# brech1/keaki

Hardware: AMD Instinct MI355X
Metric: BN254 G1 scalar-mults/sec on 2^24-point MSM (per GPU) (higher is better)
Workload: dtype u32 limbs, 256-bit Montgomery modular integer (9 x 29-bit lazy limbs in the bucket kernel, 8 x 32 elsewhere)

## Files before the change

### keaki_amd/csrc/msm.hip.h

```cpp
#pragma once
#include <type_traits>
#include "bn254_curve.hip.h"
#include "fq29.hip.h"
#include "xyzz29.hip.h"
#include "jac29.hip.h"
#include "xyzz29_g2.hip.h"

namespace bn254 {

typedef uint16_t u16;
typedef u32 v4u_t __attribute__((ext_vector_type(4)));
constexpr u32 DIGIT_NONE = 0xFFFFFFFFu;
#ifndef STAMP
#define STAMP(cond, i) do { } while (0)
#endif

struct MsmShape {
  u32 n;
  u32 c;
  u32 W;
  u32 k;
  u32 stride;
};
KDEV u32 msm_width(const MsmShape& s, u32 w) { return w < s.k ? s.c : s.c - 1; }
// ... 750 lines not shown
  for (u32 sid = blockIdx.x; sid < total; sid += gridDim.x) {
    const u32 slot = hv_owner[sid];
    const u32 t = hv_bucket[slot];
    const u32 cnt = counts[t];
    const u32 lo = (sid - hv_first[slot]) * HEAVY_SLICE, hi = min(cnt, lo + HEAVY_SLICE);
    const BinMeta bm = v.bins[part_bin(v.ps, t)];
    Xyzz<F> acc = xyzz_inf<F>();
    u32 vbase = 0;
    for (u32 cb = 0; cb < bm.nch && vbase < hi; cb += 256) {
      const u32 c = cb + threadIdx.x;
      u32 s = 0, e = 0;
      if (c < bm.nch) { const u32 se = seg_word(v, t, bm, c); s = se & 0xFFFFu; e = se >> 16; }
      const u32 len = e - s;
      u32 tot;
      const u32 v0 = vbase + block_exclusive_scan(len, &tot), v1 = v0 + len;
      if (threadIdx.x == 0) nlist = 0;
      __syncthreads();
      if (len && v1 > lo && v0 < hi) {
        const u32 a0 = v0 > lo ? v0 : lo, a1 = v1 < hi ? v1 : hi;
        const u32 k = atomicAdd(&nlist, 1u);
        seg_pos[k] = bm.img_base + c * C2_CAP + s + (a0 - v0);
        seg_n[k] = a1 - a0;
      }
      __syncthreads();
      const u32 nl = nlist;
      for (u32 j = 0; j < nl; j++) {
        const u32 p0 = seg_pos[j], nn = seg_n[j];
        for (u32 q = threadIdx.x; q < nn; q += 256) {
          u32 en = v.sorted[p0 + q];
          Aff<F> p = points[en & 0x7FFFFFFFu];
          acc = xyzz_add_mixed(acc, aff_cneg(p, (en >> 31) != 0));
        }
      }
      __syncthreads();
      vbase += tot;
    }
    sh[threadIdx.x] = acc;
    __syncthreads();
    for (u32 o2 = 128; o2 > 0; o2 >>= 1) {
      if (threadIdx.x < o2) sh[threadIdx.x] = xyzz_add(sh[threadIdx.x], sh[threadIdx.x + o2]);
      __syncthreads();
    }
    if (threadIdx.x == 0) slices[sid] = sh[0];
    __syncthreads();
  }
}
struct Acc29 {
  v4u_t q[9];
};
KDEV void acc29_store(Acc29* dst, const U29& X, const U29& Y, const U29& ZZ, const U29& ZZZ, bool empty) {
  u32 w[36];
#pragma unroll
  for (int i = 0; i < 9; i++) { w[i] = empty ? 0u : X.l[i]; w[9 + i] = empty ? 0u : Y.l[i]; w[18 + i] = empty ? 0u : ZZ.l[i]; w[27 + i] = empty ? 0u : ZZZ.l[i]; }
#pragma unroll
  for (int i = 0; i < 9; i++) dst->q[i] = v4u_t{w[4 * i], w[4 * i + 1], w[4 * i + 2], w[4 * i + 3]};
}
KDEV bool acc29_load(const Acc29* src, U29& X, U29& Y, U29& ZZ, U29& ZZZ) {
  u32 w[36];
#pragma unroll
  for (int i = 0; i < 9; i++) { const v4u_t v = src->q[i]; w[4 * i] = v[0]; w[4 * i + 1] = v[1]; w[4 * i + 2] = v[2]; w[4 * i + 3] = v[3]; }
  u32 any = 0;
#pragma unroll
  for (int i = 0; i < 9; i++) { X.l[i] = w[i]; Y.l[i] = w[9 + i]; ZZ.l[i] = w[18 + i]; ZZZ.l[i] = w[27 + i]; any |= w[18 + i]; }
  return any == 0;
}
enum { HV_SET = 0, HV_ADD = 1, HV_SET29 = 2, HV_ADD29 = 3 };
template <class F>
__global__ void __launch_bounds__(64) k_msm_heavy_combine(const u32* __restrict__ counts, const HeavyList* __restrict__ hv, u32 hv_cap, u32 hv_slice_cap,
                                                          const u32* __restrict__ hv_bucket, const u32* __restrict__ hv_first,
                                                          const Xyzz<F>* __restrict__ slices, Xyzz<F>* __restrict__ buckets, u32 mode,
                                                          Acc29* __restrict__ state29) {
  __shared__ Xyzz<F> sh[64];
  const u32 nh = min(hv->n, hv_cap);
  for (u32 slot = blockIdx.x; slot < nh; slot += gridDim.x) {
    const u32 t = hv_bucket[slot], first = hv_first[slot];
    const u32 nsl = (counts[t] + HEAVY_SLICE - 1) / HEAVY_SLICE;
    Xyzz<F> acc = xyzz_inf<F>();
    for (u32 k = threadIdx.x; k < nsl; k += 64)
      if (first + k < hv_slice_cap) acc = xyzz_add(acc, slices[first + k]);
    sh[threadIdx.x] = acc;
    __syncthreads();
    for (u32 o = 32; o > 0; o >>= 1) {
      if (threadIdx.x < o) sh[threadIdx.x] = xyzz_add(sh[threadIdx.x], sh[threadIdx.x + o]);
      __syncthreads();
    }
    if (threadIdx.x == 0) {
      Xyzz<F> r = sh[0];
      if (mode == HV_ADD) r = xyzz_add(buckets[t], r);
      if constexpr (std::is_same<F, Fq>::value) {
        if (mode == HV_ADD29) {
          U29 X, Y, ZZ, ZZZ;
          if (!acc29_load(state29 + t, X, Y, ZZ, ZZZ)) r = xyzz_add(Xyzz<Fq>{u29_to_fq(X), u29_to_fq(Y), u29_to_fq(ZZ), u29_to_fq(ZZZ)}, r);
        }
        if (mode == HV_SET29 || mode == HV_ADD29)
          acc29_store(state29 + t, u29_from_fq(r.x), u29_from_fq(r.y), u29_from_fq(r.zz), u29_from_fq(r.zzz), xyzz_is_inf(r));
        else
          buckets[t] = r;
      } else {
        buckets[t] = r;
      }
    }
    __syncthreads();
  }
}
KDEV bool msm_bucket_is_heavy(u32 cnt) { return cnt >= HEAVY_MIN; }

template <class F>
__global__ void __launch_bounds__(256) k_msm_accumulate(const Aff<F>* __restrict__ points, SortView v, const u32* __restrict__ counts,
                                                        const u32* __restrict__ perm, u32 nbuckets_total, Xyzz<F>* __restrict__ buckets, u32 cont) {
  u32 lane = blockIdx.x * blockDim.x + threadIdx.x;
  if (lane >= nbuckets_total) return;
  u32 t = perm[lane];
  u32 cnt = counts[t];
  if (msm_bucket_is_heavy(cnt)) return;
  if (cont && cnt == 0) return;
  SegWalker sw;
  seg_init(sw, v, t);
  Xyzz<F> acc = xyzz_inf<F>();
  if (cont) acc = buckets[t];
  for (u32 k = 0; k < cnt; k++) {
    u32 e = seg_next(sw, v);
    Aff<F> p = points[e & 0x7FFFFFFFu];
    acc = xyzz_add_mixed(acc, aff_cneg(p, (e >> 31) != 0));
  }
  buckets[t] = acc;
}

template <int NT>
KDEV Aff<Fq> msm_load_row(const Aff<Fq>* __restrict__ p) {
  if constexpr (NT == 0) {
    return *p;
  } else {
    const v4u_t* s = reinterpret_cast<const v4u_t*>(p);
    const v4u_t w0 = __builtin_nontemporal_load(s), w1 = __builtin_nontemporal_load(s + 1), w2 = __builtin_nontemporal_load(s + 2),
                w3 = __builtin_nontemporal_load(s + 3);
    Aff<Fq> q;
#pragma unroll
    for (int i = 0; i < 4; i++) { q.x.l[i] = w0[i]; q.x.l[4 + i] = w1[i]; q.y.l[i] = w2[i]; q.y.l[4 + i] = w3[i]; }
    return q;
  }
}
#ifdef KEAKI_DIAG
static __global__ void k_diag_mask_rows(u32* __restrict__ sorted, size_t words, u32 mask) {
  for (size_t i = (size_t)blockIdx.x * blockDim.x + threadIdx.x; i < words; i += (size_t)gridDim.x * blockDim.x) {
    const u32 e = sorted[i];
    sorted[i] = (e & 0x80000000u) | (e & mask);
  }
}
#endif
enum { ACC_WHOLE = 0, ACC_FIRST = 1, ACC_MIDDLE = 2, ACC_LAST = 3 };
template <int NT, int MODE, int PF = 2>
static __global__ void __launch_bounds__(256, 3) k_msm_accumulate_g1_u29(const Aff<Fq>* __restrict__ points, SortView v,
                                                                      const u32* __restrict__ counts, const u32* __restrict__ perm,
                                                                      u32 nbuckets_total, Xyzz<Fq>* __restrict__ buckets,
                                                                      Acc29* __restrict__ state29) {
  u32 lane = blockIdx.x * blockDim.x + threadIdx.x;
  if (lane >= nbuckets_total) return;
  u32 t = perm[lane];
  u32 cnt = counts[t];
  if constexpr (MODE == ACC_LAST) {
    if (msm_bucket_is_heavy(cnt)) cnt = 0;
  } else {
    if (msm_bucket_is_heavy(cnt)) return;
  }
  if constexpr (MODE == ACC_MIDDLE) {
    if (cnt == 0) return;
  }
  SegWalker sw;
  SegWalkerQ sq;
  if constexpr (PF != 2) seg_init(sw, v, t);
  U29 X1, Y1, ZZ, ZZZ;
  bool empty = true;
  if constexpr (MODE == ACC_MIDDLE || MODE == ACC_LAST) empty = acc29_load(state29 + t, X1, Y1, ZZ, ZZZ);
  u32 e1 = 0, e2 = 0;
  Aff<Fq> q1;
  __shared__ __attribute__((aligned(16))) u32 idx_slots[PF == 2 ? IDXQ_NQ * IDXQ_PLANE : 4];
  __shared__ __attribute__((aligned(16))) u32 idx_park[PF == 2 ? 256 * SEGQ_PARK : 4];
  const u32* my_slot = idx_slots + threadIdx.x * 4;
  u32* wave_slots = idx_slots + (threadIdx.x & ~63u) * 4;
  u32* park = idx_park + threadIdx.x * SEGQ_PARK;
  if constexpr (PF == 2) {
    segq_init(sq, v, t, park);
    if (cnt > 0) {
      segq_advance(sq, v, t, park);
      segq_fetch(sq, v, wave_slots);
      asm volatile("s_waitcnt vmcnt(0)" ::: "memory");
      e1 = segq_next(sq, v, t, my_slot, wave_slots, park);
      if (cnt > 1) {
        asm volatile("s_waitcnt vmcnt(0)" ::: "memory");
        e2 = segq_next(sq, v, t, my_slot, wave_slots, park);
      }
    }
    q1 = msm_load_row<NT>(points + (e1 & 0x7FFFFFFFu));
  } else if constexpr (PF != 0) {
    e1 = cnt > 0 ? seg_next(sw, v) : 0u; e2 = cnt > 1 ? seg_next(sw, v) : 0u;
    q1 = msm_load_row<NT>(points + (e1 & 0x7FFFFFFFu));
  }
  for (u32 k = 0; k < cnt; k++) {
    u32 e;
    Aff<Fq> q;
    if constexpr (PF == 2) {
      e = e1;
      asm volatile("s_waitcnt vmcnt(0)" ::: "memory");
      q = q1;
#pragma unroll
      for (int i = 0; i < 8; i++) { asm volatile("" : "+v"(q.x.l[i])); asm volatile("" : "+v"(q.y.l[i])); }
      u32 e3 = 0;
      if (k + 2 < cnt) e3 = segq_next(sq, v, t, my_slot, wave_slots, park);
      e1 = e2;
      if (k + 1 < cnt) q1 = msm_load_row<NT>(points + (e1 & 0x7FFFFFFFu));
      e2 = e3;
    } else if constexpr (PF != 0) {
      e = e1;
      q = q1;
      e1 = e2;
      if (k + 1 < cnt) q1 = msm_load_row<NT>(points + (e1 & 0x7FFFFFFFu));
      if (k + 2 < cnt) e2 = seg_next(sw, v);
    } else {
      e = seg_next(sw, v);
      q = msm_load_row<NT>(points + (e & 0x7FFFFFFFu));
    }
    if (aff_is_inf(q)) continue;
    q.y = f_cneg(q.y, (e >> 31) != 0);
    const U29 X2 = u29_from_sat_shift5(q.x.l), Y2 = u29_from_sat_shift5(q.y.l);
    if (empty) {
      X1 = u29_mul(X2, u29_one());
      Y1 = u29_mul(Y2, u29_one());
      ZZ = u29_one();
      ZZZ = u29_one();
      empty = false;
      continue;
    }
    const U29 U2 = u29_mul(X2, ZZ), S2 = u29_mul(Y2, ZZZ);
    const U29 P = u29_sub(U2, X1, Q29::K16), R = u29_sub(S2, Y1, Q29::K4);
    if (u29_maybe_zero(P)) {
      if (u29_is_zero(P)) {
        if (u29_is_zero(R)) {
          Xyzz<Fq> d = xyzz_dbl_aff(q);
          X1 = u29_from_fq(d.x); Y1 = u29_from_fq(d.y); ZZ = u29_from_fq(d.zz); ZZZ = u29_from_fq(d.zzz);
        } else {
          empty = true;
        }
        continue;
      }
    }
    const U29 PP = u29_sqr(P), PPP = u29_mul(P, PP), Q = u29_mul(X1, PP);
    const U29 X3 = u29_sub3(u29_sqr(R), PPP, Q);
    const U29 T = u29_sub(Q, X3, Q29::K16);
    U29 NY1;
#pragma unroll
    for (int i = 0; i < 9; i++) NY1.l[i] = Q29::K2[i] - Y1.l[i];
    Y1 = u29_mul2(R, T, NY1, PPP);
    X1 = X3;
    ZZ = u29_mul(ZZ, PP);
    ZZZ = u29_mul(ZZZ, PPP);
  }
  u32 ts = t;
  asm volatile("" : "+v"(ts));
  if constexpr (MODE == ACC_FIRST || MODE == ACC_MIDDLE) {
    acc29_store(state29 + ts, X1, Y1, ZZ, ZZZ, empty);
  } else {
    Xyzz<Fq> out = xyzz_inf<Fq>();
    if (!empty) {
      out.x = u29_to_fq(X1); out.y = u29_to_fq(Y1); out.zz = u29_to_fq(ZZ); out.zzz = u29_to_fq(ZZZ);
    }
    buckets[ts] = out;
  }
}

template <int CONT>
static __global__ void __launch_bounds__(256, 2) k_msm_accumulate_g2_u29(const Aff<Fq2>* __restrict__ points, SortView v,
                                                                      const u32* __restrict__ counts, const u32* __restrict__ perm,
                                                                      u32 nbuckets_total, Xyzz<Fq2>* __restrict__ buckets) {
  u32 lane = blockIdx.x * blockDim.x + threadIdx.x;
  if (lane >= nbuckets_total) return;
  u32 t = perm[lane];
  u32 cnt = counts[t];
  if (msm_bucket_is_heavy(cnt)) return;
  if (CONT && cnt == 0) return;
  __shared__ __attribute__((aligned(16))) u32 idx_slots[IDXQ_NQ * IDXQ_PLANE];
  __shared__ __attribute__((aligned(16))) u32 idx_park[256 * SEGQ_PARK];
  const u32* my_slot = idx_slots + threadIdx.x * 4;
  u32* wave_slots = idx_slots + (threadIdx.x & ~63u) * 4;
  u32* park = idx_park + threadIdx.x * SEGQ_PARK;
  SegWalkerQ sq;
  segq_init(sq, v, t, park);
  X29G2 acc = x29g2_inf();
  if constexpr (CONT != 0) acc = x29g2_load(buckets[t]);
  if (cnt > 0) {
    segq_advance(sq, v, t, park);
    segq_fetch(sq, v, wave_slots);
  }
  for (u32 k = 0; k < cnt; k++) {
    asm volatile("s_waitcnt vmcnt(0)" ::: "memory");
    const u32 e = segq_next(sq, v, t, my_slot, wave_slots, park);
    Aff<Fq2> q = points[e & 0x7FFFFFFFu];
    x29g2_add_mixed(acc, aff_cneg(q, (e >> 31) != 0));
  }
  u32 ts = t;
  asm volatile("" : "+v"(ts));
  buckets[ts] = x29g2_store(acc);
}

template <class F>
__global__ void __launch_bounds__(64) k_msm_reduce(const Xyzz<F>* __restrict__ buckets, MsmShape s, u32 L, u32 chunks_per_window,
                                                   Xyzz<F>* __restrict__ partials) {
  u32 g = blockIdx.x * blockDim.x + threadIdx.x;
  if (g >= s.W * chunks_per_window) return;
  u32 w = g / chunks_per_window, t = g % chunks_per_window;
  u32 lo = t * L;
  const u32 Bw = msm_nbuckets(s, w);
  const Xyzz<F>* bk = buckets + msm_bucket_base(s, w);
  typedef TailOps<F> O;
  typename O::P run = O::inf(), ws = O::inf();
  for (u32 j = L; j-- > 0;) {
    if (lo + j < Bw) {
      run = O::add(run, O::load(bk[lo + j]));
      ws = O::add(ws, run);
    }
  }
  if (lo != 0 && lo < Bw) {
    typename O::P m = O::inf();
    for (int b = 31 - __clz(lo); b >= 0; b--) {
      m = O::dbl(m);
      if ((lo >> b) & 1) m = O::add(m, run);
    }
    ws = O::add(ws, m);
  }
  partials[g] = O::store(ws);
}

template <class F>
__global__ void __launch_bounds__(64) k_msm_partial_groups(const Xyzz<F>* __restrict__ in, u32 chunks_in, u32 G, u32 chunks_out,
                                                           Xyzz<F>* __restrict__ out) {
  typedef TailOps<F> O;
  __shared__ typename O::P sh[64];
  u32 w = blockIdx.y, x = blockIdx.x, l = threadIdx.x;
  typename O::P acc = O::inf();
  for (u32 t = x * G + l; t < (x + 1) * G && t < chunks_in; t += 64) acc = O::add(acc, O::load(in[(size_t)w * chunks_in + t]));
  sh[l] = acc;
  __syncthreads();
  for (u32 o = 32; o > 0; o >>= 1) {
    if (l < o) sh[l] = O::add(sh[l], sh[l + o]);
    __syncthreads();
  }
  if (l == 0) out[(size_t)w * chunks_out + x] = O::store(sh[0]);
}

template <class F> KDEV void store_norm_jac(F* out, const Xyzz<F>& p);
template <class F>
__global__ void __launch_bounds__(64) k_msm_window_finish(const Xyzz<F>* __restrict__ partials, MsmShape s, u32 chunks_per_window,
                                                          Xyzz<F>* __restrict__ window_sums, F* __restrict__ out_jac) {
  typedef TailOps<F> O;
  __shared__ typename O::P sh[64];
  u32 w = blockIdx.x, l = threadIdx.x;
  typename O::P acc = O::inf();
  for (u32 t = l; t < chunks_per_window; t += 64) acc = O::add(acc, O::load(partials[(size_t)w * chunks_per_window + t]));
  sh[l] = acc;
  __syncthreads();
  for (u32 o = 32; o > 0; o >>= 1) {
    if (l < o) sh[l] = O::add(sh[l], sh[l + o]);
    __syncthreads();
  }
  if (l == 0) {
    typename O::P r = sh[0];
    for (u32 k = 0, nd = msm_bit_offset(s, w); k < nd; k++) r = O::dbl(r);
    if (out_jac) store_norm_jac(out_jac, O::store(r));
    else window_sums[w] = O::store(r);
  }
}

template <class F> KDEV Aff<F> xyzz_to_aff_tail(const Xyzz<F>& p) { return xyzz_to_aff(p); }
template <> KDEV Aff<Fq> xyzz_to_aff_tail<Fq>(const Xyzz<Fq>& p) {
  if (xyzz_is_inf(p)) return aff_inf<Fq>();
  Fq izzz = fq_inv(p.zzz);
  Fq izz = fq_sqr(izzz) * fq_sqr(p.zz);
  return {p.x * izz, p.y * izzz};
}
template <class F>
KDEV void store_norm_jac(F* out, const Xyzz<F>& p) {
  Aff<F> a = xyzz_to_aff_tail(p);
  if (xyzz_is_inf(p)) {
    out[0] = f_one<F>(); out[1] = f_one<F>(); out[2] = f_zero<F>();
  } else {
    out[0] = a.x; out[1] = a.y; out[2] = f_one<F>();
  }
}
template <class F>
__global__ void __launch_bounds__(64) k_msm_final(const Xyzz<F>* __restrict__ window_sums, u32 W, F* __restrict__ out_jac) {
  if (threadIdx.x != 0 || blockIdx.x != 0) return;
  Xyzz<F> acc = xyzz_inf<F>();
  for (u32 w = 0; w < W; w++) acc = xyzz_add(acc, window_sums[w]);
  store_norm_jac(out_jac, acc);
}


template <class F>
__global__ void __launch_bounds__(64) k_msm_build_tables(const Aff<F>* __restrict__ points, u32 N, MsmShape s, Aff<F>* __restrict__ table) {
  u32 i = blockIdx.x * blockDim.x + threadIdx.x;
  if (i >= N) return;
  Aff<F> p = points[i];
  table[i] = p;
#pragma unroll 1
  for (u32 w = 1; w < s.W; w++) {
    Jac<F> j = jac_from_aff(p);
    for (u32 d = msm_width(s, w - 1); d > 0; d--) j = jac_dbl(j);
    p = jac_to_aff(j);
    table[(size_t)w * N + i] = p;
  }
}

constexpr u32 TABLE_MAX_W = 16;
static __global__ void __launch_bounds__(64) k_msm_build_tables_g1(const Aff<Fq>* __restrict__ points, u32 N, MsmShape s, Aff<Fq>* __restrict__ table) {
  u32 i = blockIdx.x * blockDim.x + threadIdx.x;
  if (i >= N) return;
  const Aff<Fq> p = points[i];
  table[i] = p;
  if (aff_is_inf(p)) {
    for (u32 w = 1; w < s.W; w++) table[(size_t)w * N + i] = p;
    return;
  }
  J29 j;
  j.x = u29_from_fq(p.x); j.y = u29_from_fq(p.y); j.z = u29_one();
  U29 zs[TABLE_MAX_W];
  U29 prod = u29_one();
#pragma unroll 1
  for (u32 w = 1; w < s.W; w++) {
    for (u32 d = msm_width(s, w - 1); d > 0; d--) j = j29_dbl(j);
    Aff<Fq> tmp = {u29_to_fq(j.x), u29_to_fq(j.y)};
    table[(size_t)w * N + i] = tmp;
#pragma unroll
    for (u32 k = 1; k < TABLE_MAX_W; k++) if (k == w) zs[k] = j.z;
    prod = u29_mul(prod, j.z);
  }
  U29 tinv = u29_from_fq(fq_inv(u29_to_fq(prod)));
#pragma unroll 1
  for (u32 w = s.W - 1; w >= 1; w--) {
    U29 pre = u29_one(), zw = u29_one();
#pragma unroll
    for (u32 k = 1; k < TABLE_MAX_W; k++) {
      if (k < w) pre = u29_mul(pre, zs[k]);
      if (k == w) zw = zs[k];
    }
    const U29 zinv = u29_mul(tinv, pre);
    tinv = u29_mul(tinv, zw);
    const U29 zi2 = u29_sqr(zinv), zi3 = u29_mul(zi2, zinv);
    const Aff<Fq> jxy = table[(size_t)w * N + i];
    Aff<Fq> a = {u29_to_fq(u29_mul(u29_from_sat_shift5(jxy.x.l), zi2)), u29_to_fq(u29_mul(u29_from_sat_shift5(jxy.y.l), zi3))};
    table[(size_t)w * N + i] = a;
  }
}

template <class F>
__global__ void __launch_bounds__(64) k_sum_jac(const F* __restrict__ pts, u32 k, F* __restrict__ out_jac) {
  if (threadIdx.x != 0 || blockIdx.x != 0) return;
  Xyzz<F> acc = xyzz_inf<F>();
  for (u32 i = 0; i < k; i++) {
    Jac<F> p = {pts[3 * i], pts[3 * i + 1], pts[3 * i + 2]};
    if (jac_is_inf(p)) continue;
    Aff<F> a = f_eq(p.z, f_one<F>()) ? Aff<F>{p.x, p.y} : jac_to_aff(p);
    acc = xyzz_add_mixed(acc, a);
  }
  store_norm_jac(out_jac, acc);
}

}
```

### keaki_amd/csrc/msm_host.hip.h

```cpp
#pragma once
#include <algorithm>
#include <functional>
#include <type_traits>
#include <vector>
#include "internal.h"
#include "msm.hip.h"

namespace keaki_internal {
using namespace bn254;

inline int choose_window(size_t n, int forced = 0) {
  if (forced >= 3 && forced <= 24) return forced;
  if (n < 32) return 3;
  double best = 1e300;
  int bc = 3;
  for (int c = 3; c <= 22; c++) {
    MsmPlan p = msm_make_plan(n, c);
    if (p.nb > ((size_t)PART_MAX_BINS << PART_MAX_FINE_SHIFT)) continue;
    double cost = (double)n * p.s.W + 2.8 * (double)p.nb;
    if ((double)p.nb < 131072.0) cost *= 131072.0 / (double)p.nb;
    if (cost < best) { best = cost; bc = c; }
  }
  return bc;
}

template <class F>
keaki_status msm_dev(keaki_hip_ctx* ctx, const Aff<F>* d_points, size_t srs_len, const void* d_scalars, size_t n, void* d_out_jac,
                     const Aff<F>* d_table = nullptr, int c_table = 0, const MsmPipe* pipe = nullptr) {
  if (!d_out_jac || (n && (!d_points || !d_scalars))) return fail(ctx, KEAKI_ERR_BAD_ARG, "msm: null pointer");
  if (n > srs_len) return fail(ctx, KEAKI_ERR_TOO_LARGE, "msm: %zu scalars but the SRS holds %zu points", n, srs_len);
  if (n >= (1ull << 31)) return fail(ctx, KEAKI_ERR_BAD_ARG, "msm: n must be < 2^31 per device");
  const bool shared = d_table != nullptr && (n * 2 > srs_len || ctx->tune.msm_short_tables != 0);
  const MsmPlan plan = shared ? msm_make_plan(n, c_table) : msm_make_plan(n, choose_window(n, ctx->tune.msm_c));
  MsmShape s = plan.s;
  MsmShape rs = s;
  size_t nb = plan.nb;
  if (shared) {
    s.stride = (u32)srs_len;
    u32 cr = 0;
    while ((1u << cr) < plan.max_b) cr++;
    rs.n = s.n; rs.c = cr; rs.W = 1; rs.k = 1; rs.stride = 0;
    nb = plan.max_b;
    d_points = d_table;
    if ((double)srs_len * s.W >= 2147483647.0) return fail(ctx, KEAKI_ERR_BAD_ARG, "msm: precomputed table index overflows 31 bits");
  }
  ctx->last_c = (int)s.c;
  if ((double)n * s.W >= 4294967295.0) return fail(ctx, KEAKI_ERR_BAD_ARG, "msm: n * windows overflows 32-bit positions");
  u32 L = sizeof(F) > sizeof(Fq) ? (plan.max_b >= 64 ? 8 : plan.max_b)
                                 : plan.max_b >= (1u << 21) ? 32 : plan.max_b >= (1u << 20) ? 16 : (plan.max_b >= 64 ? 8 : plan.max_b);
  if (ctx->tune.reduce_l >= 1 && ctx->tune.reduce_l <= 4096 && (u32)ctx->tune.reduce_l <= plan.max_b) L = (u32)ctx->tune.reduce_l;
  const u32 chunks = cdiv(plan.max_b, L);
  ST_TRY(reserve(ctx, ctx->wsums, (size_t)rs.W * sizeof(Xyzz<F>)));
  Xyzz<F>* wsums = (Xyzz<F>*)ctx->wsums.p;
  F* out = (F*)d_out_jac;
  hipStream_t st = ctx->stream;
  if (ctx->timing) (void)hipEventRecord(ctx->ev[0], st);
  if (n == 0) {
    hipLaunchKernelGGL((k_msm_final<F>), dim3(1), dim3(64), 0, st, (const Xyzz<F>*)wsums, 0u, out);
    return launch_check(ctx, "msm_final");
  }
  const size_t K = pipe ? pipe->ranges.size() : 1;
  if (pipe && K < 1) return fail(ctx, KEAKI_ERR_BAD_ARG, "msm: bad chunk bounds");
  struct Pass {
    size_t lo, m, pairs, max_chunks, cm_bytes, bt_bytes, bm_bytes, sg_bytes, ts_bytes;
    PartShape ps;
  };
  std::vector<Pass> passes(K);
  size_t w_digits = 0, w_sorted = 0, w_offsets = 0, w_cursor = 0, w_pairs = 0, w_total = 0;
  for (size_t j = 0; j < K; j++) {
    Pass& q = passes[j];
    q.lo = pipe ? pipe->ranges[j].first : 0;
    q.m = pipe ? pipe->ranges[j].second : n;
    if (q.m == 0 || q.lo > n || q.m > n - q.lo) return fail(ctx, KEAKI_ERR_BAD_ARG, "msm: bad chunk bounds");
    w_total += q.m;
    if (!part_make_shape(q.m, s.W, nb, &q.ps, ctx->tune.part_shift))
      return fail(ctx, KEAKI_ERR_BAD_ARG, "msm: %zu buckets / %u windows exceed the bucket sort's LDS budget (window too large)", nb, s.W);
    q.pairs = q.m * (size_t)s.W;
    q.max_chunks = part_max_chunks(q.pairs, q.ps.nbins);
    q.cm_bytes = (size_t)q.ps.nbins * q.ps.ntiles * sizeof(uint2);
    q.bt_bytes = ((size_t)q.ps.nbins * 4 + 15) & ~(size_t)15;
    q.bm_bytes = (size_t)q.ps.nbins * sizeof(BinMeta);
    q.sg_bytes = nb * sizeof(v4u_t);
    q.ts_bytes = (size_t)q.ps.ntiles * (q.ps.nbins + 1) * 2;
    w_digits = std::max(w_digits, (size_t)q.ps.ntiles * q.ps.te * 4);
    w_sorted = std::max(w_sorted, q.pairs * 4 + 64);
    w_offsets = std::max(w_offsets, q.max_chunks * q.ps.nf * 4);
    w_cursor = std::max(w_cursor, q.cm_bytes + q.bt_bytes + q.bm_bytes + q.sg_bytes + q.ts_bytes);
    w_pairs = std::max(w_pairs, q.pairs);
  }
  if (w_total != n) return fail(ctx, KEAKI_ERR_BAD_ARG, "msm: the chunks cover %zu of %zu pairs", w_total, n);
  bool u29 = false;
  if constexpr (std::is_same<F, Fq>::value) u29 = ctx->tune.acc_u29;
  if constexpr (std::is_same<F, Fq2>::value) u29 = ctx->tune.acc_u29_g2;
  bool lazy_state = K > 1 && u29 && std::is_same<F, Fq>::value;
  ST_TRY(reserve(ctx, ctx->digits, w_digits));
  ST_TRY(reserve(ctx, ctx->sorted, w_sorted));
  ST_TRY(reserve(ctx, ctx->hist, nb * 4));
  ST_TRY(reserve(ctx, ctx->offsets, w_offsets));
  ST_TRY(reserve(ctx, ctx->cursor, w_cursor));
  ST_TRY(reserve(ctx, ctx->buckets, nb * sizeof(Xyzz<F>)));
  ST_TRY(reserve(ctx, ctx->partials, ((size_t)rs.W * chunks + (size_t)rs.W * 256) * sizeof(Xyzz<F>)));
  ST_TRY(reserve(ctx, ctx->perm, nb * 4 + 2 * CNT_BINS * 4 + sizeof(HeavyList)));
  const u32 hv_cap = (u32)(w_pairs / HEAVY_MIN + 1), hv_slice_cap = (u32)(hv_cap + w_pairs / HEAVY_SLICE + 1);
  const size_t hv_hdr = ((2 * (size_t)hv_cap + hv_slice_cap) * 4 + 255) & ~(size_t)255;
  ST_TRY(reserve(ctx, ctx->heavy, hv_hdr + (size_t)hv_slice_cap * sizeof(Xyzz<F>)));
  if (lazy_state) {
    const keaki_status st29 = reserve(ctx, ctx->acc29, nb * sizeof(Acc29));
    if (st29 == KEAKI_ERR_OOM) { lazy_state = false; u29 = false; ctx->err.clear(); }
    else if (st29 != KEAKI_OK) return st29;
  }
  u32 *tiles = (u32*)ctx->digits.p, *sorted = (u32*)ctx->sorted.p, *hist = (u32*)ctx->hist.p;
  u32* segoff = (u32*)ctx->offsets.p;
  Xyzz<F>* buckets = (Xyzz<F>*)ctx->buckets.p;
  Xyzz<F>* partials = (Xyzz<F>*)ctx->partials.p;
  Acc29* state29 = lazy_state ? (Acc29*)ctx->acc29.p : nullptr;
  u32* perm = (u32*)ctx->perm.p;
  u32 *gstart = perm + nb, *ghist = gstart + CNT_BINS;
  HeavyList* hv = (HeavyList*)(ghist + CNT_BINS);
  u32 *hv_bucket = (u32*)ctx->heavy.p, *hv_first = hv_bucket + hv_cap, *hv_owner = hv_first + hv_cap;
  Xyzz<F>* hv_slices = (Xyzz<F>*)((char*)ctx->heavy.p + hv_hdr);
  for (size_t j = 0; j < K; j++) {
    const Pass& q = passes[j];
    const PartShape& ps = q.ps;
    if (pipe && pipe->stage) ST_TRY(pipe->stage(j));
    MsmShape sj = s;
    sj.n = (u32)q.m;
    const Fr* scal = (const Fr*)d_scalars + q.lo;
    const Aff<F>* pts = d_points + q.lo;
    const bool first = j == 0, last = j + 1 == K;
    uint2* cellmeta = (uint2*)ctx->cursor.p;
    u32* bin_total = (u32*)((char*)ctx->cursor.p + q.cm_bytes);
    BinMeta* bins = (BinMeta*)((char*)bin_total + q.bt_bytes);
    v4u_t* segtab = (v4u_t*)((char*)bins + q.bm_bytes);
    u16* tstart = (u16*)((char*)segtab + q.sg_bytes);
    {
      const dim3 g1(ps.ntiles < ctx->n_cu ? ps.ntiles : ctx->n_cu), b1(T1_THREADS);
#define KEAKI_TILE_SORT(WS) hipLaunchKernelGGL(k_tile_sort<WS>, g1, b1, 0, st, scal, sj, ps, tiles, tstart)
      switch (s.W) {
        case 11: KEAKI_TILE_SORT(11); break;
        case 12: KEAKI_TILE_SORT(12); break;
        case 13: KEAKI_TILE_SORT(13); break;
        case 14: KEAKI_TILE_SORT(14); break;
        case 15: KEAKI_TILE_SORT(15); break;
        case 16: KEAKI_TILE_SORT(16); break;
        default: KEAKI_TILE_SORT(0); break;
      }
#undef KEAKI_TILE_SORT
    }
    ST_TRY(launch_check(ctx, "tile_sort"));
    hipLaunchKernelGGL(k_cell_prefix, dim3(ps.nbins), dim3(1024), 0, st, (const u16*)tstart, ps, cellmeta, bin_total);
    hipLaunchKernelGGL(k_bin_scan, dim3(1), dim3(1024), 0, st, (const u32*)bin_total, ps.nbins, bins);
    {
#define KEAKI_CHUNK_SORT1(L, R, Q, M)                                                                                                                  \
  hipLaunchKernelGGL((k_chunk_sort<L, R, Q, M>), dim3(ps.nbins), dim3(C2_THREADS), 0, st, (const u32*)tiles, (const uint2*)cellmeta, (const BinMeta*)bins, sj, \
                     ps, (u32)nb, sorted, segtab, segoff, hist)
#define KEAKI_CHUNK_SORT(L, R, Q) do { if (ctx->tune.cs_masked) KEAKI_CHUNK_SORT1(L, R, Q, true); else KEAKI_CHUNK_SORT1(L, R, Q, false); } while (0)
      switch (ps.geom) {
        case 0: KEAKI_CHUNK_SORT(8, 1, 16); break;
        case 1: KEAKI_CHUNK_SORT(16, 1, 16); break;
        case 2: KEAKI_CHUNK_SORT(16, 2, 8); break;
        default: KEAKI_CHUNK_SORT(16, 4, 4); break;
      }
#undef KEAKI_CHUNK_SORT1
#undef KEAKI_CHUNK_SORT
    }
    ST_TRY(launch_check(ctx, "chunk_sort"));
#ifdef KEAKI_DIAG
    if (ctx->tune.diag_row_mask) hipLaunchKernelGGL(k_diag_mask_rows, dim3(4096), dim3(256), 0, st, sorted, (size_t)q.pairs, (u32)ctx->tune.diag_row_mask);
#endif
    const SortView view = {sorted, bins, segtab, segoff, ps};
    HIP_TRY(ctx, hipMemsetAsync(ghist, 0, CNT_BINS * 4 + sizeof(HeavyList), st));
    hipLaunchKernelGGL(k_cnt_hist, dim3(cdiv(nb, 1024)), dim3(256), 0, st, (const u32*)hist, (u32)nb, ghist, hv, hv_cap, hv_slice_cap, hv_bucket, hv_first,
                       hv_owner);
    hipLaunchKernelGGL(k_cnt_offsets, dim3(1), dim3(CNT_BINS), 0, st, (const u32*)ghist, gstart);
    hipLaunchKernelGGL(k_cnt_scatter, dim3(cdiv(nb, 1024)), dim3(256), 0, st, (const u32*)hist, (u32)nb, gstart, perm);
    ST_TRY(launch_check(ctx, "cnt_sort"));
    if (ctx->timing && last) (void)hipEventRecord(ctx->ev[1], st);
    const dim3 ga(cdiv(nb, 256)), ba(256);
    bool done = false;
    if constexpr (std::is_same<F, Fq>::value) {
      if (u29) {
#define KEAKI_ACC(NT, MODE) hipLaunchKernelGGL((k_msm_accumulate_g1_u29<NT, MODE>), ga, ba, 0, st, pts, view, (const u32*)hist, (const u32*)perm, (u32)nb, buckets, state29)
        if (K == 1) {
          if (ctx->tune.acc_nt) KEAKI_ACC(1, ACC_WHOLE);
          else if (!ctx->tune.acc_prefetch)
            hipLaunchKernelGGL((k_msm_accumulate_g1_u29<0, ACC_WHOLE, 0>), ga, ba, 0, st, pts, view, (const u32*)hist, (const u32*)perm, (u32)nb, buckets, state29);
          else if (!ctx->tune.acc_idxq)
            hipLaunchKernelGGL((k_msm_accumulate_g1_u29<0, ACC_WHOLE, 1>), ga, ba, 0, st, pts, view, (const u32*)hist, (const u32*)perm, (u32)nb, buckets, state29);
          else KEAKI_ACC(0, ACC_WHOLE);
        }
        else if (first) KEAKI_ACC(0, ACC_FIRST);
        else if (!last) KEAKI_ACC(0, ACC_MIDDLE);
        else KEAKI_ACC(0, ACC_LAST);
#undef KEAKI_ACC
        done = true;
      }
    }
    if constexpr (std::is_same<F, Fq2>::value) {
      if (u29) {
        if (first) hipLaunchKernelGGL(k_msm_accumulate_g2_u29<0>, ga, ba, 0, st, pts, view, (const u32*)hist, (const u32*)perm, (u32)nb, buckets);
        else hipLaunchKernelGGL(k_msm_accumulate_g2_u29<1>, ga, ba, 0, st, pts, view, (const u32*)hist, (const u32*)perm, (u32)nb, buckets);
        done = true;
      }
    }
    if (!done)
      hipLaunchKernelGGL((k_msm_accumulate<F>), ga, ba, 0, st, pts, view, (const u32*)hist, (const u32*)perm, (u32)nb, buckets, first ? 0u : 1u);
    ST_TRY(launch_check(ctx, "msm_accumulate"));
    const u32 hv_mode = lazy_state && !last ? (first ? HV_SET29 : HV_ADD29) : (first ? HV_SET : HV_ADD);
    hipLaunchKernelGGL((k_msm_heavy<F>), dim3(HEAVY_GRID), dim3(256), 0, st, pts, view, (const u32*)hist,
                       (const HeavyList*)hv, hv_slice_cap, (const u32*)hv_bucket, (const u32*)hv_first, (const u32*)hv_owner, hv_slices);
    hipLaunchKernelGGL((k_msm_heavy_combine<F>), dim3(HEAVY_COMBINE_GRID), dim3(64), 0, st, (const u32*)hist, (const HeavyList*)hv, hv_cap, hv_slice_cap,
                       (const u32*)hv_bucket, (const u32*)hv_first, (const Xyzz<F>*)hv_slices, buckets, hv_mode, state29);
    ST_TRY(launch_check(ctx, "msm_heavy"));
  }
  if (ctx->timing) (void)hipEventRecord(ctx->ev[2], st);
  hipLaunchKernelGGL((k_msm_reduce<F>), dim3(cdiv((size_t)rs.W * chunks, 64)), dim3(64), 0, st, (const Xyzz<F>*)buckets, rs, L, chunks, partials);
  const Xyzz<F>* fin_in = partials;
  u32 fin_chunks = chunks;
  if (chunks > 256) {
    const u32 G = cdiv(chunks, 128);
    const u32 chunks2 = cdiv(chunks, G);
    Xyzz<F>* partials2 = partials + (size_t)rs.W * chunks;
    hipLaunchKernelGGL((k_msm_partial_groups<F>), dim3(chunks2, rs.W), dim3(64), 0, st, (const Xyzz<F>*)partials, chunks, G, chunks2, partials2);
    fin_in = partials2; fin_chunks = chunks2;
  }
  hipLaunchKernelGGL((k_msm_window_finish<F>), dim3(rs.W), dim3(64), 0, st, fin_in, rs, fin_chunks, wsums, rs.W == 1 ? out : (F*)nullptr);
  if (rs.W != 1) hipLaunchKernelGGL((k_msm_final<F>), dim3(1), dim3(64), 0, st, (const Xyzz<F>*)wsums, rs.W, out);
  ST_TRY(launch_check(ctx, "msm_reduce/final"));
  if (ctx->timing) {
    (void)hipEventRecord(ctx->ev[3], st);
    ctx->timing_pending = true;
  }
  return KEAKI_OK;
}

template <class F>
keaki_status msm_build_tables(keaki_hip_ctx* ctx, const Aff<F>* d_points, size_t N, int c_table, Aff<F>* d_table) {
  MsmPlan plan = msm_make_plan(N, c_table);
  bool done = false;
  if constexpr (std::is_same<F, Fq>::value) {
    if (plan.s.W <= TABLE_MAX_W) {
      hipLaunchKernelGGL(k_msm_build_tables_g1, dim3(cdiv(N, 64)), dim3(64), 0, ctx->stream, d_points, (u32)N, plan.s, d_table);
      done = true;
    }
  }
  if (!done)
  hipLaunchKernelGGL((k_msm_build_tables<F>), dim3(cdiv(N, 64)), dim3(64), 0, ctx->stream, d_points, (u32)N, plan.s, d_table);
  return launch_check(ctx, "msm_build_tables");
}
inline int choose_window_shared(size_t n, int forced = 0) {
  if (forced >= 3 && forced <= 24) return forced;
  double best = 1e300;
  int bc = 8;
  for (int c = 8; c <= 23; c++) {
    MsmPlan p = msm_make_plan(n, c);
    if (p.max_b > ((size_t)PART_MAX_BINS << PART_MAX_FINE_SHIFT)) continue;
    double cost = (double)n * p.s.W + 2.8 * (double)p.max_b;
    if ((double)p.max_b < 131072.0) cost *= 131072.0 / (double)p.max_b;
    if (cost < best) { best = cost; bc = c; }
  }
  return bc;
}
inline u32 msm_plan_windows(size_t n, int c) { return msm_make_plan(n, c).s.W; }

}
```

Before: 1.023 billion.

## Replace running-sum bucket reduction with bit-decomposed row/column line sums

Replaces the per-chunk running-sum bucket reduction with a bit-decomposition scheme. Bucket indices are laid out as a 2D grid, and partial row and column line sums are computed and then combined. For each bit of the index, the lines whose coordinate has that bit set are summed and doubled the matching number of times. This avoids the serial run/ws chains and the per-chunk double-and-add correction, and exposes more parallelism in the reduction tail. The cost is four kernel launches and a different partial buffer layout, with a new tunable T reusing the reduce_l knob.

```diff
diff --git a/keaki_amd/csrc/msm.hip.h b/keaki_amd/csrc/msm.hip.h
--- a/keaki_amd/csrc/msm.hip.h
+++ b/keaki_amd/csrc/msm.hip.h
@@ -1076,72 +1076,117 @@
   buckets[ts] = x29g2_store(acc);
 }
 
+struct TailGeom {
+  u32 lb, h;
+  u32 nr, nc;
+  u32 tr, tc;
+  u32 gc, gf;
+  u32 sc, sr;
+  u32 o_pr, o_c, o_r, o_u, per_w;
+};
+constexpr u32 TAIL_LINE_LANES = 16;
+inline TailGeom tail_geom(u32 max_b, u32 t) {
+  TailGeom g;
+  g.lb = 0;
+  while ((1u << g.lb) < max_b) g.lb++;
+  g.h = (g.lb + 1) / 2;
+  g.nr = 1u << (g.lb - g.h); g.nc = 1u << g.h;
+  g.tr = t < g.nr ? t : g.nr; g.tc = t < g.nc ? t : g.nc;
+  g.gc = (g.nr + g.tr - 1) / g.tr; g.gf = (g.nc + g.tc - 1) / g.tc;
+  g.sc = 1; while (g.sc * 2 <= g.gc && g.sc < TAIL_LINE_LANES) g.sc *= 2;
+  g.sr = 1; while (g.sr * 2 <= g.gf && g.sr < TAIL_LINE_LANES) g.sr *= 2;
+  g.o_pr = g.nc * g.gc; g.o_c = g.o_pr + g.nr * g.gf; g.o_r = g.o_c + g.nc; g.o_u = g.o_r + g.nr; g.per_w = g.o_u + g.lb + 1;
+  return g;
+}
+KDEV u32 tree_top(u32 m) { return m <= 1 ? 0u : 1u << (31 - __clz(m - 1)); }
+KDEV u32 umin(u32 a, u32 b) { return a < b ? a : b; }
+
 template <class F>
-__global__ void __launch_bounds__(64) k_msm_reduce(const Xyzz<F>* __restrict__ buckets, MsmShape s, u32 L, u32 chunks_per_window,
-                                                   Xyzz<F>* __restrict__ partials) {
-  u32 g = blockIdx.x * blockDim.x + threadIdx.x;
-  if (g >= s.W * chunks_per_window) return;
-  u32 w = g / chunks_per_window, t = g % chunks_per_window;
-  u32 lo = t * L;
+__global__ void __launch_bounds__(64) k_msm_tail_lines(const Xyzz<F>* __restrict__ buckets, MsmShape s, TailGeom g, Xyzz<F>* __restrict__ ws) {
+  typedef TailOps<F> O;
+  const u32 t = blockIdx.x * 64 + threadIdx.x, w = blockIdx.y;
+  if (t >= g.o_c) return;
+  u32 j0, step, len;
+  if (t < g.o_pr) {
+    const u32 b = t & (g.nc - 1), r0 = (t >> g.h) * g.tr;
+    j0 = (r0 << g.h) + b; step = g.nc; len = umin(g.tr, g.nr - r0);
+  } else {
+    const u32 u = t - g.o_pr, a = u & (g.nr - 1), c0 = (u >> (g.lb - g.h)) * g.tc;
+    j0 = (a << g.h) + c0; step = 1; len = umin(g.tc, g.nc - c0);
+  }
   const u32 Bw = msm_nbuckets(s, w);
-  const Xyzz<F>* bk = buckets + msm_bucket_base(s, w);
-  typedef TailOps<F> O;
-  typename O::P run = O::inf(), ws = O::inf();
-  for (u32 j = L; j-- > 0;) {
-    if (lo + j < Bw) {
-      run = O::add(run, O::load(bk[lo + j]));
-      ws = O::add(ws, run);
-    }
-  }
-  if (lo != 0 && lo < Bw) {
-    typename O::P m = O::inf();
-    for (int b = 31 - __clz(lo); b >= 0; b--) {
-      m = O::dbl(m);
-      if ((lo >> b) & 1) m = O::add(m, run);
-    }
-    ws = O::add(ws, m);
-  }
-  partials[g] = O::store(ws);
+  len = j0 >= Bw ? 0u : umin(len, (Bw - j0 + step - 1) / step);
+  const Xyzz<F>* bk = buckets + msm_bucket_base(s, w) + j0;
+  typename O::P acc = O::inf();
+  for (u32 i = 0; i < len; i++) acc = O::add(acc, O::load(bk[(size_t)i * step]));
+  ws[(size_t)w * g.per_w + t] = O::store(acc);
 }
 
 template <class F>
-__global__ void __launch_bounds__(64) k_msm_partial_groups(const Xyzz<F>* __restrict__ in, u32 chunks_in, u32 G, u32 chunks_out,
-                                                           Xyzz<F>* __restrict__ out) {
+__global__ void __launch_bounds__(64) k_msm_tail_line_sums(TailGeom g, Xyzz<F>* __restrict__ ws) {
   typedef TailOps<F> O;
   __shared__ typename O::P sh[64];
-  u32 w = blockIdx.y, x = blockIdx.x, l = threadIdx.x;
+  const u32 l = threadIdx.x, cb = (g.nc * g.sc + 63) / 64;
+  const bool col = blockIdx.x < cb;
+  const u32 span = col ? g.sc : g.sr, np = col ? g.gc : g.gf, nl = col ? g.nc : g.nr;
+  const u32 q = (col ? blockIdx.x : blockIdx.x - cb) * 64 + l, line = q / span, k = q % span;
+  Xyzz<F>* base = ws + (size_t)blockIdx.y * g.per_w;
+  const Xyzz<F>* in = base + (col ? 0u : g.o_pr);
   typename O::P acc = O::inf();
-  for (u32 t = x * G + l; t < (x + 1) * G && t < chunks_in; t += 64) acc = O::add(acc, O::load(in[(size_t)w * chunks_in + t]));
+  if (line < nl)
+    for (u32 i = k; i < np; i += span) acc = O::add(acc, O::load(in[(size_t)i * nl + line]));
   sh[l] = acc;
   __syncthreads();
-  for (u32 o = 32; o > 0; o >>= 1) {
+  for (u32 o = span >> 1; o > 0; o >>= 1) {
+    if (k < o) sh[l] = O::add(sh[l], sh[l + o]);
+    __syncthreads();
+  }
+  if (k == 0 && line < nl) base[(col ? g.o_c : g.o_r) + line] = O::store(sh[l]);
+}
+
+constexpr u32 TAIL_BITS_THREADS = 256;
+template <class F>
+__global__ void __launch_bounds__(TAIL_BITS_THREADS) k_msm_tail_bits(MsmShape s, TailGeom g, Xyzz<F>* __restrict__ ws) {
+  typedef TailOps<F> O;
+  __shared__ typename O::P sh[TAIL_BITS_THREADS];
+  const u32 e = blockIdx.x, w = blockIdx.y, l = threadIdx.x;
+  Xyzz<F>* base = ws + (size_t)w * g.per_w;
+  const bool colside = e < g.h, all = e == g.lb;
+  const Xyzz<F>* in = base + (colside ? g.o_c : g.o_r);
+  const u32 bit = colside ? e : e - g.h, cnt = all ? g.nr : (colside ? g.nc : g.nr) >> 1;
+  typename O::P acc = O::inf();
+  for (u32 i = l; i < cnt; i += TAIL_BITS_THREADS) {
+    const u32 x = all ? i : ((i >> bit) << (bit + 1)) | (1u << bit) | (i & ((1u << bit) - 1u));
+    acc = O::add(acc, O::load(in[x]));
+  }
+  sh[l] = acc;
+  __syncthreads();
+  for (u32 o = tree_top(umin(cnt, TAIL_BITS_THREADS)); o > 0; o >>= 1) {
     if (l < o) sh[l] = O::add(sh[l], sh[l + o]);
     __syncthreads();
   }
-  if (l == 0) out[(size_t)w * chunks_out + x] = O::store(sh[0]);
+  if (l == 0) {
+    typename O::P r = sh[0];
+    for (u32 d = (all ? 0u : e) + msm_bit_offset(s, w); d > 0; d--) r = O::dbl(r);
+    base[g.o_u + e] = O::store(r);
+  }
 }
 
 template <class F> KDEV void store_norm_jac(F* out, const Xyzz<F>& p);
 template <class F>
-__global__ void __launch_bounds__(64) k_msm_window_finish(const Xyzz<F>* __restrict__ partials, MsmShape s, u32 chunks_per_window,
-                                                          Xyzz<F>* __restrict__ window_sums, F* __restrict__ out_jac) {
+__global__ void __launch_bounds__(64) k_msm_tail_final(TailGeom g, u32 W, const Xyzz<F>* __restrict__ ws, F* __restrict__ out_jac) {
   typedef TailOps<F> O;
   __shared__ typename O::P sh[64];
-  u32 w = blockIdx.x, l = threadIdx.x;
+  const u32 l = threadIdx.x, per = g.lb + 1, cnt = W * per;
   typename O::P acc = O::inf();
-  for (u32 t = l; t < chunks_per_window; t += 64) acc = O::add(acc, O::load(partials[(size_t)w * chunks_per_window + t]));
+  for (u32 i = l; i < cnt; i += 64) acc = O::add(acc, O::load(ws[(size_t)(i / per) * g.per_w + g.o_u + i % per]));
   sh[l] = acc;
   __syncthreads();
-  for (u32 o = 32; o > 0; o >>= 1) {
+  for (u32 o = tree_top(umin(cnt, 64u)); o > 0; o >>= 1) {
     if (l < o) sh[l] = O::add(sh[l], sh[l + o]);
     __syncthreads();
   }
-  if (l == 0) {
-    typename O::P r = sh[0];
-    for (u32 k = 0, nd = msm_bit_offset(s, w); k < nd; k++) r = O::dbl(r);
-    if (out_jac) store_norm_jac(out_jac, O::store(r));
-    else window_sums[w] = O::store(r);
-  }
+  if (l == 0) store_norm_jac(out_jac, O::store(sh[0]));
 }
 
 template <class F> KDEV Aff<F> xyzz_to_aff_tail(const Xyzz<F>& p) { return xyzz_to_aff(p); }
@@ -1160,15 +1205,6 @@
     out[0] = a.x; out[1] = a.y; out[2] = f_one<F>();
   }
 }
-template <class F>
-__global__ void __launch_bounds__(64) k_msm_final(const Xyzz<F>* __restrict__ window_sums, u32 W, F* __restrict__ out_jac) {
-  if (threadIdx.x != 0 || blockIdx.x != 0) return;
-  Xyzz<F> acc = xyzz_inf<F>();
-  for (u32 w = 0; w < W; w++) acc = xyzz_add(acc, window_sums[w]);
-  store_norm_jac(out_jac, acc);
-}
-
-
 template <class F>
 __global__ void __launch_bounds__(64) k_msm_build_tables(const Aff<F>* __restrict__ points, u32 N, MsmShape s, Aff<F>* __restrict__ table) {
   u32 i = blockIdx.x * blockDim.x + threadIdx.x;
diff --git a/keaki_amd/csrc/msm_host.hip.h b/keaki_amd/csrc/msm_host.hip.h
--- a/keaki_amd/csrc/msm_host.hip.h
+++ b/keaki_amd/csrc/msm_host.hip.h
@@ -46,17 +46,14 @@
   }
   ctx->last_c = (int)s.c;
   if ((double)n * s.W >= 4294967295.0) return fail(ctx, KEAKI_ERR_BAD_ARG, "msm: n * windows overflows 32-bit positions");
-  u32 L = sizeof(F) > sizeof(Fq) ? (plan.max_b >= 64 ? 8 : plan.max_b)
-                                 : plan.max_b >= (1u << 21) ? 32 : plan.max_b >= (1u << 20) ? 16 : (plan.max_b >= 64 ? 8 : plan.max_b);
-  if (ctx->tune.reduce_l >= 1 && ctx->tune.reduce_l <= 4096 && (u32)ctx->tune.reduce_l <= plan.max_b) L = (u32)ctx->tune.reduce_l;
-  const u32 chunks = cdiv(plan.max_b, L);
-  ST_TRY(reserve(ctx, ctx->wsums, (size_t)rs.W * sizeof(Xyzz<F>)));
-  Xyzz<F>* wsums = (Xyzz<F>*)ctx->wsums.p;
+  u32 T = 22;
+  if (ctx->tune.reduce_l >= 1 && ctx->tune.reduce_l <= 4096) T = (u32)ctx->tune.reduce_l;
+  const TailGeom tg = tail_geom(plan.max_b, T);
   F* out = (F*)d_out_jac;
   hipStream_t st = ctx->stream;
   if (ctx->timing) (void)hipEventRecord(ctx->ev[0], st);
   if (n == 0) {
-    hipLaunchKernelGGL((k_msm_final<F>), dim3(1), dim3(64), 0, st, (const Xyzz<F>*)wsums, 0u, out);
+    hipLaunchKernelGGL((k_msm_tail_final<F>), dim3(1), dim3(64), 0, st, tg, 0u, (const Xyzz<F>*)nullptr, out);
     return launch_check(ctx, "msm_final");
   }
   const size_t K = pipe ? pipe->ranges.size() : 1;
@@ -99,7 +96,7 @@
   ST_TRY(reserve(ctx, ctx->offsets, w_offsets));
   ST_TRY(reserve(ctx, ctx->cursor, w_cursor));
   ST_TRY(reserve(ctx, ctx->buckets, nb * sizeof(Xyzz<F>)));
-  ST_TRY(reserve(ctx, ctx->partials, ((size_t)rs.W * chunks + (size_t)rs.W * 256) * sizeof(Xyzz<F>)));
+  ST_TRY(reserve(ctx, ctx->partials, (size_t)rs.W * tg.per_w * sizeof(Xyzz<F>)));
   ST_TRY(reserve(ctx, ctx->perm, nb * 4 + 2 * CNT_BINS * 4 + sizeof(HeavyList)));
   const u32 hv_cap = (u32)(w_pairs / HEAVY_MIN + 1), hv_slice_cap = (u32)(hv_cap + w_pairs / HEAVY_SLICE + 1);
   const size_t hv_hdr = ((2 * (size_t)hv_cap + hv_slice_cap) * 4 + 255) & ~(size_t)255;
@@ -112,7 +109,6 @@
   u32 *tiles = (u32*)ctx->digits.p, *sorted = (u32*)ctx->sorted.p, *hist = (u32*)ctx->hist.p;
   u32* segoff = (u32*)ctx->offsets.p;
   Xyzz<F>* buckets = (Xyzz<F>*)ctx->buckets.p;
-  Xyzz<F>* partials = (Xyzz<F>*)ctx->partials.p;
   Acc29* state29 = lazy_state ? (Acc29*)ctx->acc29.p : nullptr;
   u32* perm = (u32*)ctx->perm.p;
   u32 *gstart = perm + nb, *ghist = gstart + CNT_BINS;
@@ -214,19 +210,12 @@
     ST_TRY(launch_check(ctx, "msm_heavy"));
   }
   if (ctx->timing) (void)hipEventRecord(ctx->ev[2], st);
-  hipLaunchKernelGGL((k_msm_reduce<F>), dim3(cdiv((size_t)rs.W * chunks, 64)), dim3(64), 0, st, (const Xyzz<F>*)buckets, rs, L, chunks, partials);
-  const Xyzz<F>* fin_in = partials;
-  u32 fin_chunks = chunks;
-  if (chunks > 256) {
-    const u32 G = cdiv(chunks, 128);
-    const u32 chunks2 = cdiv(chunks, G);
-    Xyzz<F>* partials2 = partials + (size_t)rs.W * chunks;
-    hipLaunchKernelGGL((k_msm_partial_groups<F>), dim3(chunks2, rs.W), dim3(64), 0, st, (const Xyzz<F>*)partials, chunks, G, chunks2, partials2);
-    fin_in = partials2; fin_chunks = chunks2;
-  }
-  hipLaunchKernelGGL((k_msm_window_finish<F>), dim3(rs.W), dim3(64), 0, st, fin_in, rs, fin_chunks, wsums, rs.W == 1 ? out : (F*)nullptr);
-  if (rs.W != 1) hipLaunchKernelGGL((k_msm_final<F>), dim3(1), dim3(64), 0, st, (const Xyzz<F>*)wsums, rs.W, out);
-  ST_TRY(launch_check(ctx, "msm_reduce/final"));
+  Xyzz<F>* tws = (Xyzz<F>*)ctx->partials.p;
+  hipLaunchKernelGGL((k_msm_tail_lines<F>), dim3(cdiv(tg.o_c, 64), rs.W), dim3(64), 0, st, (const Xyzz<F>*)buckets, rs, tg, tws);
+  hipLaunchKernelGGL((k_msm_tail_line_sums<F>), dim3(cdiv((size_t)tg.nc * tg.sc, 64) + cdiv((size_t)tg.nr * tg.sr, 64), rs.W), dim3(64), 0, st, tg, tws);
+  hipLaunchKernelGGL((k_msm_tail_bits<F>), dim3(tg.lb + 1, rs.W), dim3(TAIL_BITS_THREADS), 0, st, rs, tg, tws);
+  hipLaunchKernelGGL((k_msm_tail_final<F>), dim3(1), dim3(64), 0, st, tg, rs.W, (const Xyzz<F>*)tws, out);
+  ST_TRY(launch_check(ctx, "msm_tail"));
   if (ctx->timing) {
     (void)hipEventRecord(ctx->ev[3], st);
     ctx->timing_pending = true;
```

After: 1.031 billion (median of 6 runs). No clear change (+0.7%).
